# xieydd/crane-scheduler

Hardware: AMD Instinct MI355X
Metric: placements/sec (higher is better)
Workload: dtype f64

## Files before the change

crane-scheduler_amd/csrc/k1stream.hip:

```cpp
#include <hip/hip_runtime.h>

#include "k1stream_body.hpp"

namespace crane {

template <int PD, int PR, bool FULL>
__global__ __launch_bounds__(256) __attribute__((amdgpu_waves_per_eu(PD * PR <= 24 ? K1S_WAVES : 1)))
void k1_stream_steps(K1Args a, K1Step step) {
    __shared__ K1Lds<PD, PR> lds;
    k1_stream_body<PD, PR, FULL, (int)sizeof(K1Args) + (int)sizeof(K1Step)>(a, step, blockIdx.x, gridDim.x, lds);
}

template <int PD, int PR, bool FULL = false>
static hipError_t launch_t(const K1Args& a, const K1Step& sa, hipStream_t st) {
    const unsigned grid = (unsigned)((a.N + 255) / 256);
    return klaunch("k1_stream_steps", k1_stream_steps<PD, PR, FULL>, dim3(grid), dim3(256), 0, st, a, sa);
}

hipError_t launch_stream_steps(int pd, int pr, const K1Args& a, const K1Step& sa, hipStream_t st) {
    if (a.N <= 0) return hipSuccess;
    if (K1S_FULL && a.pol.npd == 4 && a.pol.npr == 6 && a.pol.n_win == kFullWin) return launch_t<4, 6, true>(a, sa, st);
    if (pd <= 4 && pr <= 6) return launch_t<4, 6>(a, sa, st);
    if (pd <= 8 && pr <= 8) return launch_t<8, 8>(a, sa, st);
    return launch_t<16, 16>(a, sa, st);
}

}
```

crane-scheduler_amd/csrc/k1stream_body.hpp:

```cpp
#pragma once
#include <hip/hip_runtime.h>

#include <cstddef>

#include "dyn_types.hpp"
#include "kernels.hpp"
#include "node_rec.hpp"
#include "step_node.hpp"

namespace crane {

#ifndef K1S_SKIP
#define K1S_SKIP 0
#endif
#ifndef K1S_TAIL1
#define K1S_TAIL1 1
#endif
#ifndef K1S_WAVES
#define K1S_WAVES 7
#endif
#ifndef K1S_KWARM
#define K1S_KWARM 1
#endif
#ifndef K1S_FULL
#define K1S_FULL 1
#endif
#ifndef K1S_SREC
#define K1S_SREC 64
#endif
#ifndef K1S_SCAP
#define K1S_SCAP 128
#endif
#ifndef K1S_RTAIL
#define K1S_RTAIL 1
#endif
#ifndef K1S_SMALL
#define K1S_SMALL 32
#endif
constexpr int kSRec = K1S_SREC;
constexpr int kSCap = K1S_SCAP;
constexpr int kSmallTail = K1S_SMALL;
static_assert(kSmallTail <= 32 && kSmallTail <= kSCap, "one record per lane of a half wave, staged in LDS");

template <int PD, int PR>
__device__ __forceinline__ void emit_task(const NodeRec<PD, PR>& r, int64_t n, int q, const int32_t* dw, int64_t tmin,
                                          int64_t tmax, double wsum, int32_t noprio, const StepTables& st,
                                          int64_t blk, const S1Out& s1o, double winv) {
    constexpr int NB = PR + 2, F = PR + 1;
    int64_t c[NB];
#pragma unroll
    for (int k = 0; k < PR; ++k) c[k] = r.e_prio[k];
    c[PR] = r.e_hv;
    c[F] = r.e_fail;
    uint32_t inm = 0;
#pragma unroll
    for (int k = 0; k < NB; ++k) inm |= (c[k] > tmin && c[k] <= tmax) ? 1u << k : 0u;
    if (!((inm >> q) & 1u)) return;
    const int cnt0 = __builtin_popcount(inm), cnt1 = __builtin_popcount(inm & ~(1u << F));
    int64_t cq = c[0];
#pragma unroll
    for (int j = 1; j < NB; ++j) cq = q == j ? c[j] : cq;
    int rk0 = 0;
    bool fb = false;
    int64_t cn1 = INT64_MAX, cn0;
#pragma unroll
    for (int j = 0; j < NB; ++j) {
        const bool in = (inm >> j) & 1u;
        const bool before = in && (c[j] < cq || (c[j] == cq && j < q));
        const bool after = in && (c[j] > cq || (c[j] == cq && j > q));
        rk0 += before;
        if (j == F) {
            fb = before;
            cn0 = after ? min(cn1, c[j]) : cn1;
        } else {
            cn1 = after ? min(cn1, c[j]) : cn1;
        }
    }
    const int rk1 = rk0 - (fb ? 1 : 0);
    double tk[PR];
#pragma unroll
    for (int k = 0; k < PR; ++k) tk[k] = r.t[k];
    double ssum = 0.0;
#pragma unroll
    for (int k = 0; k < PR; ++k) ssum = cq < c[k] ? ssum + tk[k] : ssum;
    const int64_t pk = pack_key(score_of_sum(ssum, cq < c[PR] ? r.pen : 0, wsum, noprio, winv), n);
    const int64_t pk0 = pack_key(dw[5], n);
#pragma unroll
    for (int T = 0; T < 2; ++T) {
        const int32_t slot = dw[T ? 2 : 0];
        if (slot < 0 || (T == 1 && q == F)) continue;
        const int rk = T ? rk1 : rk0, cnt = T ? cnt1 : cnt0;
        const int64_t cn = T ? cn1 : cn0;
        const int32_t kq = (int32_t)((T == 1 || !(cq < r.e_fail)) ? pk : -1);
        const int32_t kt = (int32_t)((T == 1 || !(tmin < r.e_fail)) ? pk0 : -1);
        const bool multi = ((dw[4] >> T) & 1) != 0;
        if (!multi) {
            if (rk == 0) {
                Step1 v;
                v.bp = cq;
                v.k0 = kt;
                v.k1 = kq;
                s1o.put(T, slot, v);
            }
            continue;
        }
        if (rk + 1 < cnt) {
            Mid pc;
            pc.s = cq;
            pc.e = cn;
            pc.key = kq;
            pc.pad = 0;
            (st.mid + (int64_t)T * st.mpad + blk * st.mstride + dw[T ? 3 : 1])[rk] = pc;
        }
        if (rk == 0) {
            Step1 x;
            x.bp = cq;
            x.k0 = kt;
            x.k1 = -1;
            s1o.put(T, slot, x);
        }
        if (rk == cnt - 1) {
            Step1 y;
            y.bp = cq;
            y.k0 = -1;
            y.k1 = kq;
            s1o.put(T, slot + 1, y);
        }
    }
}

template <int BS, class Rec>
__device__ __forceinline__ void tail(bool g1, Rec* lrec, Step1* s1l, Step1* srt, StepShared& ssh, const K1Step& step,
                                     int64_t blk, unsigned long long* trace, int64_t wg) {
    constexpr int kPc = ((int)(kSRec * sizeof(Rec)) / PieceScr::bytes_per_piece) & ~3;
    const PieceScr ps{reinterpret_cast<unsigned char*>(lrec), (K1S_SKIP & 8) ? 0 : (kPc < 128 ? kPc : 128)};
#if K1S_SKIP & 16
    StepTables st = step.st;
    st.rows = nullptr;
#else
    const StepTables& st = step.st;
#endif
    step_epilogue<BS, kSCap>(g1, s1l, srt, ssh, st, blk, nullptr, ps, trace, wg);
    CRANE_TSTAMP(trace, wg, 4);
}

template <bool ONE>
__device__ __forceinline__ void small_tail_bounds(const StepTables& st, int64_t (&pre)[2]) {
    const int lane = threadIdx.x & 63;
    const int T0 = ONE ? 0 : __builtin_amdgcn_readfirstlane((int)(threadIdx.x >> 6));
    pre[0] = small_tile_bound(st, T0, 0, lane);
    pre[1] = ONE ? small_tile_bound(st, 1, 0, lane) : 0;
}
template <bool ONE>
__device__ __forceinline__ void small_tail(const Step1* s1l, int32_t n0, int32_t n1, const StepShared& ssh,
                                           const K1Step& step, int64_t blk, const int64_t (&pre)[2], bool rows,
                                           unsigned long long* trace, int64_t wg) {
    constexpr int NK = ONE ? 2 : 1;
    const StepTables& st = step.st;
    const int lane = threadIdx.x & 63;
    const int T0 = ONE ? 0 : __builtin_amdgcn_readfirstlane((int)(threadIdx.x >> 6));
    const int tl = lane < 32 ? lane : 64;
    int32_t n[NK], fl[NK];
    Step1 r[NK];
    SmallScan sc[NK];
#pragma unroll
    for (int k = 0; k < NK; ++k) {
        const int T = T0 + k;
        n[k] = __builtin_amdgcn_readfirstlane(T ? n1 : n0);
        fl[k] = block_flat_max<256>(ssh, T);
        r[k].bp = 0;
        r[k].k0 = r[k].k1 = -1;
        if (lane < n[k]) r[k] = s1l[T * kSCap + lane];
    }
#pragma unroll
    for (int k = 0; k < NK; ++k) sc[k] = small_scan(r[k], n[k], lane < 32 ? r[k].bp : pre[k], tl);
#pragma unroll
    for (int k = 0; k < NK; ++k) small_records_store(T0 + k, n[k], r[k], sc[k], st, blk);
    CRANE_TSTAMP(trace, wg, 6);
    if (rows) {
#pragma unroll
        for (int k = 0; k < NK; ++k) small_row_store(T0 + k, 0, sc[k], fl[k], st, blk);
        for (int t0 = 16; t0 < st.ntiles; t0 += 16) {
#pragma unroll
            for (int k = 0; k < NK; ++k) {
                const SmallScan s = small_scan(r[k], n[k], small_tile_bound(st, T0 + k, t0, lane), 64);
                small_row_store(T0 + k, t0, s, fl[k], st, blk);
            }
        }
    }
    CRANE_TSTAMP(trace, wg, 4);
}

constexpr int kFullWin = 2;
template <int PD, int PR>
struct K1Lds {
    alignas(16) NodeRec<PD, PR> lrec[kSRec];
    alignas(16) Step1 s1l[2 * kSCap];
    alignas(16) Step1 srt[2 * kSCap];
    alignas(16) uint32_t xch[5][4];
    StepShared ssh;
    uint8_t rank_lane[256];
};
template <int PD, int PR, bool FULL, int WARM>
__device__ __forceinline__ void k1_stream_body(const K1Args& a, const K1Step& step, const int64_t wg, const int64_t nwg,
                                               K1Lds<PD, PR>& lds) {
    using Rec = NodeRec<PD, PR>;
    constexpr int BS = 256;
    const int npd = FULL ? PD : a.pol.npd, npr = FULL ? PR : a.pol.npr, nwin = FULL ? kFullWin : a.pol.n_win;
    Rec* const lrec = lds.lrec;
    uint8_t* const rank_lane = lds.rank_lane;
    Step1* const s1l = lds.s1l;
    Step1* const srt = lds.srt;
    uint32_t(*const xch)[4] = lds.xch;
    StepShared& ssh = lds.ssh;
    const DevPolicy& pol = a.pol;
    const int64_t N = a.N;
    const int64_t blk = xcd_block(wg, nwg), first = blk * BS, n = first + threadIdx.x;
    CRANE_TSTAMP(a.trace, wg, 0);
    const int lo = (int)min((int64_t)threadIdx.x, N - 1 - first);
    const int64_t bt0 = step.batch[0], bt1 = step.batch[1];
    int64_t pt[PD], qt[PR];
    double pv[PD], qv[PR];
#pragma unroll
    for (int k = 0; k < PD; ++k) {
        pt[k] = kTsInvalid;
        pv[k] = 0.0;
    }
#pragma unroll
    for (int k = 0; k < PR; ++k) {
        qt[k] = kTsInvalid;
        qv[k] = 0.0;
    }
    if (FULL || pol.n_slots > 0) {
#pragma unroll
        for (int k = 0; k < PD; ++k) {
            const int64_t row = k < npd ? pol.pred_slot[k] : 0;
            pt[k] = (a.ts + (row * N + first))[lo];
            pv[k] = (a.val + (row * N + first))[lo];
        }
#pragma unroll
        for (int k = 0; k < PR; ++k) {
            const int64_t row = k < npr ? pol.prio_slot[k] : 0;
            qt[k] = (a.ts + (row * N + first))[lo];
            qv[k] = (a.val + (row * N + first))[lo];
        }
    }
    uint32_t bc[kMaxWin];
    double hvl = 0.0;
    int64_t hvt = kTsInvalid;
    if (a.buckets) {
        const uint32_t* __restrict__ base = a.bucket_base ? a.bucket_base : a.buckets;
        uint32_t bz[kMaxWin];
#pragma unroll
        for (int b = 0; b < kMaxWin; ++b) {
            bc[b] = b < nwin ? (a.buckets + first)[(int64_t)b * N + lo] : 0u;
            bz[b] = b < nwin ? (base + first)[(int64_t)b * N + lo] : 0u;
        }
        if (a.bucket_base) bucket_anchor_counts(bz, bc);
    } else if (a.hv) {
        hvl = a.hv[first + lo];
        hvt = a.hv_ts ? a.hv_ts[first + lo] : a.hv_ts_counts;
    }
#if K1S_KWARM
    kernarg_warm<WARM>();
#endif
    const int64_t tmin = readfirstlane64(bt0), tmax = readfirstlane64(bt1);
    if (threadIdx.x < 4) ssh.lc[threadIdx.x >> 1][threadIdx.x & 1] = 0;
    CRANE_TSTAMP(a.trace, wg, 1);
    const bool valid = n < N;
    int64_t e_fail = kTsInvalid;
#pragma unroll
    for (int k = 0; k < PD; ++k) {
        const double u = pv[k], lim = pol.pred_limit[k];
        const int64_t e = sat_add(pt[k], pol.pred_dur[k]);
        const bool over = k < npd && pt[k] != kTsInvalid && !(u < 0.0) && lim != 0.0 && u > lim;
        e_fail = over ? max(e_fail, e) : e_fail;
    }
    Rec hr;
    if (a.buckets) {
        if (valid && !a.buckets_keep) {
#pragma unroll
            for (int b = 0; b < kMaxWin; ++b)
                if (b < nwin) (a.buckets + first)[(int64_t)b * N + threadIdx.x] = 0;
        }
        rec_hot_counts<PD, PR, FULL ? kFullWin : 0>(pol, bc, N, n, valid ? a.cnt_out : nullptr, valid ? a.hvc_out : nullptr,
                               a.hv_ts_counts, hr);
    } else if (a.hv) {
        rec_hot_annotation<PD, PR>(hvl, hvt, hr);
    } else {
        hr.pen = 0;
        hr.e_hv = kTsInvalid;
    }
    double s = 0.0;
    StepRange both;
    int64_t ep[PR];
    double tp[PR];
#pragma unroll
    for (int k = 0; k < PR; ++k) {
        const bool use = k < npr && qt[k] != kTsInvalid && !(qv[k] < 0.0);
        double term = (1.0 - qv[k]) * pol.prio_w[k];
        term = term * 100.0;
        const int64_t e = sat_add(qt[k], pol.prio_dur[k]);
        ep[k] = use ? e : kTsInvalid;
        tp[k] = use ? term : 0.0;
        s = tmin < ep[k] ? s + tp[k] : s;
        both.add(ep[k], tmin, tmax);
    }
    both.add(hr.e_hv, tmin, tmax);
    const int32_t s0 = score_of_sum(s, tmin < hr.e_hv ? hr.pen : 0, step.wsum, step.noprio, step.winv);
    StepRange g[2];
    StepSlots so;
    step_classify(both, e_fail, valid, s0, n, tmin, tmax, g, so);
    CRANE_TSTAMP(a.trace, wg, 2);
    const int lane = threadIdx.x & 63, wv = threadIdx.x >> 6;
    const uint32_t w0 = g[0].word(), w1 = g[1].word(), w2 = (g[0].cnt | g[1].cnt) ? 1u : 0u;
    uint32_t e0 = wave_scan_add(w0), e1 = wave_scan_add(w1), e2 = wave_scan_add(w2);
    const int32_t fm0 = wave_max(so.flat0), fm1 = wave_max(so.flat1);
    if (lane == 0) {
        ssh.fm[0][wv] = fm0;
        ssh.fm[1][wv] = fm1;
    }
    if (lane == 63) {
        xch[0][wv] = e0;
        xch[1][wv] = e1;
        xch[2][wv] = e2;
    }
    e0 -= w0;
    e1 -= w1;
    e2 -= w2;
    __syncthreads();
    uint32_t base[3], tot[3];
#pragma unroll
    for (int k = 0; k < 3; ++k) {
        const uint4 x = *reinterpret_cast<const uint4*>(xch[k]);
        base[k] = (wv > 0 ? x.x : 0u) + (wv > 1 ? x.y : 0u) + (wv > 2 ? x.z : 0u);
        tot[k] = x.x + x.y + x.z + x.w;
    }
    step_slots(g, base[0] + e0, base[1] + e1, so);
    const int32_t rs = (int32_t)(base[2] + e2);
    const int32_t nst = (int32_t)tot[2];
    if (threadIdx.x == 0) {
        ssh.lc[0][0] = (int32_t)(tot[0] & 0xFFFF);
        ssh.lc[0][1] = (int32_t)(tot[0] >> 16);
        ssh.lc[1][0] = (int32_t)(tot[1] & 0xFFFF);
        ssh.lc[1][1] = (int32_t)(tot[1] >> 16);
    }
    step_publish_store<BS>(ssh, step.st, blk, [&](int L) {
        return (int32_t)((L & 1) ? tot[L >> 1] >> 16 : tot[L >> 1] & 0xFFFF);
    });
    const bool g1 = (int32_t)max(tot[0] & 0xFFFF, tot[1] & 0xFFFF) > min(kSCap, step.st.lds_cap);
    CRANE_TSTAMP(a.trace, wg, 3);
    const S1Out s1o{s1l, step.st.stage + blk * 2 * step.st.bs, g1, (int64_t)kSCap, step.st.s1pad};
    const bool stepped = (g[0].cnt | g[1].cnt) != 0;
    auto put = [&](Rec* r) {
        r->e_fail = e_fail;
        r->pen = hr.pen;
        r->e_hv = hr.e_hv;
#pragma unroll
        for (int k = 0; k < PR; ++k) {
            r->e_prio[k] = ep[k];
            r->t[k] = tp[k];
        }
        int32_t* dw = reinterpret_cast<int32_t*>(r->e_pred);
        dw[0] = so.slot0;
        dw[1] = so.mslot0;
        dw[2] = so.slot1;
        dw[3] = so.mslot1;
        dw[4] = (so.multi0 ? 1 : 0) | (so.multi1 ? 2 : 0);
        dw[5] = s0;
    };
    if (stepped && !(K1S_SKIP & 4)) {
        rank_lane[rs] = (uint8_t)threadIdx.x;
        if (rs < kSRec) put(&lrec[rs]);
        else put(static_cast<Rec*>(step.srec) + n);
    }
    __syncthreads();
    const bool t1 = K1S_TAIL1 && (step.tail1 == 1 || (step.tail1 == 0 && nwg >= 4096));
    const bool emit1 = t1 && nst * (PR + 2) <= 64;
    if (emit1 && threadIdx.x >= 64) return;
    const int nthr = emit1 ? 64 : BS;
#if K1S_RTAIL
    const int32_t n0 = (int32_t)(tot[0] & 0xFFFF), n1 = (int32_t)(tot[1] & 0xFFFF);
    const bool small = !g1 && max(n0, n1) <= kSmallTail && !step.st.prow && !(K1S_SKIP & 2);
    const bool srows = step.st.rows && !(K1S_SKIP & 16);
    int64_t tpre[2] = {0, 0};
    if (small && srows && threadIdx.x < (t1 ? 64 : 128)) {
        if (t1) small_tail_bounds<true>(step.st, tpre);
        else small_tail_bounds<false>(step.st, tpre);
    }
#endif
    for (int32_t c0 = 0; c0 < ((K1S_SKIP & 1) ? 0 : nst); c0 += kSRec) {
        const int32_t m = min(kSRec, nst - c0);
        if (c0 > 0) {
            constexpr int W = 3 + 2 * PR + 3;
            for (int i = threadIdx.x; i < m * W; i += BS) {
                const int j = i / W, f = i - j * W;
                const int64_t* src = reinterpret_cast<const int64_t*>(static_cast<const Rec*>(step.srec) + first +
                                                                      rank_lane[c0 + j]);
                reinterpret_cast<int64_t*>(&lrec[j])[f] = src[f];
            }
            __syncthreads();
        }
        {
            constexpr int NB = PR + 2;
            for (int tk = threadIdx.x; tk < m * NB; tk += nthr) {
                const int j = tk / NB;
                int q = tk - j * NB;
                asm volatile("" : "+v"(q));
                emit_task<PD, PR>(lrec[j], first + rank_lane[c0 + j], q,
                                  reinterpret_cast<const int32_t*>(lrec[j].e_pred), tmin, tmax, step.wsum, step.noprio,
                                  step.st, blk, s1o, step.winv);
            }
        }
        __syncthreads();
    }
    CRANE_TSTAMP(a.trace, wg, 5);
    if (K1S_SKIP & 2) return;
#if K1S_RTAIL
    if (small) {
        if (threadIdx.x >= (t1 ? 64 : 128)) return;
        if (t1) small_tail<true>(s1l, n0, n1, ssh, step, blk, tpre, srows, a.trace, wg);
        else small_tail<false>(s1l, n0, n1, ssh, step, blk, tpre, srows, a.trace, wg);
        return;
    }
#endif
    if (t1) {
        if (threadIdx.x >= 64) return;
        if (threadIdx.x < 2) {
            const int T = threadIdx.x;
            ssh.fm[T][0] = block_flat_max<BS>(ssh, T);
        }
        tail<64>(g1, lrec, s1l, srt, ssh, step, blk, a.trace, wg);
        return;
    }
    tail<BS>(g1, lrec, s1l, srt, ssh, step, blk, a.trace, wg);
}

}
```

crane-scheduler_amd/csrc/lds_hash.hpp:

```cpp
#pragma once
#include <hip/hip_runtime.h>

#include <cstdint>

#include "kernels.hpp"

namespace crane {

constexpr int kDSlots = 4096;

template <int SLOTS = kDSlots>
__device__ __forceinline__ int32_t hash_add(int32_t* hkey, uint32_t* hcnt, uint32_t* hist, int bb, int32_t key,
                                            uint32_t add) {
    constexpr int kBits = __builtin_ctz(SLOTS);
    uint32_t h = ((uint32_t)key * 2654435761u) >> (32 - kBits);
    for (;;) {
        const int32_t old = atomicCAS(&hkey[h], -1, key);
        if (old == -1 || old == key) {
            atomicAdd(&hcnt[h], add);
            if (old == -1) {
                atomicAdd(&hist[(key >> 3) >> bb], 1u);
                return (int32_t)h;
            }
            return -1;
        }
        h = (h + 1) & (SLOTS - 1);
    }
}

template <int SLOTS, int KPER>
__device__ __forceinline__ uint32_t wave_aggregate(const int32_t* key, int32_t* hkey, uint32_t* hcnt, uint32_t* hist,
                                                   int bb, uint16_t* useg) {
    const int lane = threadIdx.x & 63;
    uint32_t nw = 0;
#pragma unroll
    for (int u = 0; u < KPER; ++u) {
        const bool ok = key[u] >= 0;
        const uint64_t am = __ballot(ok);
        if (am == 0) continue;
        const int lead = __ffsll((long long)am) - 1;
        const int32_t kl = __builtin_amdgcn_readlane(key[u], lead);
        const uint64_t m = __ballot(ok && key[u] == kl);
        const bool mine = lane == lead || (ok && key[u] != kl);
        const int32_t slot = mine ? hash_add<SLOTS>(hkey, hcnt, hist, bb, lane == lead ? kl : key[u],
                                                    lane == lead ? (uint32_t)__popcll(m) : 1u)
                                  : -1;
        const uint64_t nm = __ballot(slot >= 0);
        if (slot >= 0) useg[nw + __popcll(nm & ((1ull << lane) - 1ull))] = (uint16_t)slot;
        nw += __popcll(nm);
    }
    return nw;
}

constexpr int kDeltaChunk = 1024;
constexpr int delta_slots(int chunk) { return 2 * kDeltaMaxWin * chunk; }
constexpr size_t delta_lds_bytes(int chunk, int threads) {
    return sizeof(uint32_t) * 2 * (size_t)delta_slots(chunk) +
           sizeof(uint16_t) * (size_t)(threads / 64) * (size_t)(chunk / threads * kDeltaMaxWin * 64);
}

template <int BT, int CHUNK = kDeltaChunk>
__device__ __forceinline__ void k2_delta_body(const int32_t blk, const int32_t* __restrict__ bnode, int64_t N,
                                              const HotDelta& d, uint32_t* __restrict__ adj) {
    static_assert(CHUNK % BT == 0 && BT % 64 == 0, "whole bindings per lane, whole waves");
    constexpr int kSlots = delta_slots(CHUNK);
    static_assert((kSlots & (kSlots - 1)) == 0 && kSlots <= 65536, "hash_add masks the slot; uniq holds it in 16 bits");
    constexpr int kPer = CHUNK / BT;
    constexpr int kKeys = kPer * kDeltaMaxWin;
    static_assert(sizeof(uint32_t) * 2 * (size_t)kSlots + sizeof(uint16_t) * (BT / 64) * (kKeys * 64) ==
                      delta_lds_bytes(CHUNK, BT),
                  "the launchers' footprint is this layout's");
    extern __shared__ __attribute__((aligned(16))) uint32_t sh[];
    __shared__ uint32_t hist[32];
    int32_t* hkey = reinterpret_cast<int32_t*>(sh);
    uint32_t* hcnt = sh + kSlots;
    uint16_t* uniq = reinterpret_cast<uint16_t*>(hcnt + kSlots);
    const int64_t L = d.start[d.n_rng];
    int64_t pos[kPer];
    int32_t nd[kPer];
#pragma unroll
    for (int u = 0; u < kPer; ++u) {
        const int64_t t = (int64_t)blk * CHUNK + u * BT + threadIdx.x;
        int k = 0;
        for (int r = 1; r < d.n_rng; ++r) k += t >= d.start[r] ? 1 : 0;
        pos[u] = d.lo[k] + (t - d.start[k]);
        nd[u] = bnode[t < L ? pos[u] : d.lo[0]];
        if (t >= L) nd[u] = -1;
    }
    for (int i = threadIdx.x; i < kSlots; i += BT) {
        hkey[i] = -1;
        hcnt[i] = 0;
    }
    if (threadIdx.x < 32) hist[threadIdx.x] = 0;
    __syncthreads();
    int32_t key[kKeys];
#pragma unroll
    for (int u = 0; u < kPer; ++u) {
        const bool ok = nd[u] >= 0 && (int64_t)nd[u] < N;
#pragma unroll
        for (int r = 0; r < kDeltaMaxWin; ++r) {
            const bool ia = pos[u] >= d.a[r], ip = pos[u] >= d.p[r];
            key[u * kDeltaMaxWin + r] = ok && r < d.n_win && ia != ip ? ((nd[u] * 8 + r) << 1) | (ia ? 1 : 0) : -1;
        }
    }
    uint16_t* useg = uniq + (threadIdx.x >> 6) * (kKeys * 64);
    const uint32_t nw = wave_aggregate<kSlots, kKeys>(key, hkey, hcnt, hist, 24, useg);
    __syncthreads();
    for (uint32_t i = threadIdx.x & 63; i < nw; i += 64) {
        const int s = useg[i];
        const int32_t k = hkey[s];
        const uint32_t c = hcnt[s];
        atomicAdd(&adj[(int64_t)((k >> 1) & 7) * N + (k >> 4)], (k & 1) ? 0u - c : c);
    }
}


}
```

crane-scheduler_amd/csrc/pods.hpp:

```cpp
#pragma once
#include <hip/hip_runtime.h>

#include <cstdint>

#include "kernels.hpp"

namespace crane {

constexpr size_t kK3pLds = 1024 * (sizeof(uint64_t) + sizeof(uint32_t));

__device__ __forceinline__ bool pod_gt(uint64_t ka, uint32_t va, uint64_t kb, uint32_t vb) {
    return (va >> 30) != (vb >> 30) ? va > vb : (ka != kb ? ka > kb : va > vb);
}

template <int kT>
__device__ __forceinline__ void k3p_tile(const int64_t t, const PodPrep& pp, unsigned char* lds) {
    static_assert(1024 % kT == 0 && kT >= 64, "a tile is 1024 pods");
    constexpr int kU = 1024 / kT, kG = kU * (kT / 64);
    constexpr uint64_t kSign = 1ull << 63;
    __shared__ int32_t gcn[kG], gcd[kG];
    uint64_t* ku = reinterpret_cast<uint64_t*>(lds);
    uint32_t* kv = reinterpret_cast<uint32_t*>(lds + 8 * 1024);
    const int w = threadIdx.x >> 6, lane = threadIdx.x & 63;
    const int64_t pend = min(pp.P, (t + 1) * 1024);
    bool live[kU], ds[kU], inorder = true;
    int64_t tn[kU];
#pragma unroll
    for (int u = 0; u < kU; ++u) {
        const int64_t p = t * 1024 + u * kT + threadIdx.x;
        live[u] = p < pend;
        ds[u] = live[u] && pp.flags && (pp.flags[p] & 1u);
        tn[u] = live[u] ? pp.now[p] : 0;
        if (p + 1 < pend) inorder &= tn[u] <= pp.now[p + 1];
        if (live[u] && pp.keys) pp.keys[p] = -1;
    }
    int32_t e0, e1;
    if (__syncthreads_and(inorder)) {
        uint64_t mnm[kU], mdm[kU];
#pragma unroll
        for (int u = 0; u < kU; ++u) {
            mnm[u] = __ballot(live[u] && !ds[u]);
            mdm[u] = __ballot(ds[u]);
            if (lane == 0) {
                gcn[u * (kT / 64) + w] = __popcll(mnm[u]);
                gcd[u * (kT / 64) + w] = __popcll(mdm[u]);
            }
        }
        __syncthreads();
        int32_t tot_n = 0, tot_d = 0;
#pragma unroll
        for (int i = 0; i < kG; ++i) {
            tot_n += gcn[i];
            tot_d += gcd[i];
        }
        e0 = tot_n;
        e1 = tot_n + tot_d;
        const uint64_t lt = (1ull << lane) - 1ull;
#pragma unroll
        for (int u = 0; u < kU; ++u) {
            const int gi = u * (kT / 64) + w, i = u * kT + threadIdx.x;
            int32_t pre_n = 0, pre_d = 0;
            for (int k = 0; k < gi; ++k) {
                pre_n += gcn[k];
                pre_d += gcd[k];
            }
            const int pos = !live[u] ? i
                            : ds[u]  ? tot_n + pre_d + __popcll(mdm[u] & lt)
                                     : pre_n + __popcll(mnm[u] & lt);
            ku[pos] = live[u] ? (uint64_t)tn[u] ^ kSign : ~0ull;
            kv[pos] = ((live[u] ? (ds[u] ? 1u : 0u) : 2u) << 30) | (uint32_t)i;
        }
        __syncthreads();
    } else {
        e0 = e1 = 0;
#pragma unroll
        for (int u = 0; u < kU; ++u) {
            const int i = u * kT + threadIdx.x;
            ku[i] = live[u] ? (uint64_t)tn[u] ^ kSign : ~0ull;
            kv[i] = ((live[u] ? (ds[u] ? 1u : 0u) : 2u) << 30) | (uint32_t)i;
            e0 += __syncthreads_count(live[u] && !ds[u]);
            e1 += __syncthreads_count(ds[u]);
        }
        e1 += e0;
        for (int k = 2; k <= 1024; k <<= 1) {
            for (int j = k >> 1; j > 0; j >>= 1) {
                for (int q = threadIdx.x; q < 512; q += kT) {
                    const int i = ((q & ~(j - 1)) << 1) | (q & (j - 1)), l = i | j;
                    const uint64_t ka = ku[i], kb = ku[l];
                    const uint32_t va = kv[i], vb = kv[l];
                    if (pod_gt(ka, va, kb, vb) == ((i & k) == 0)) {
                        ku[i] = kb;
                        ku[l] = ka;
                        kv[i] = vb;
                        kv[l] = va;
                    }
                }
                __syncthreads();
            }
        }
    }
#pragma unroll
    for (int u = 0; u < kU; ++u) {
        const int i = u * kT + threadIdx.x;
        const uint32_t v = kv[i];
        if ((v >> 30) < 2u) {
            pp.perm[t * 1024 + i] = (int32_t)(t * 1024 + (v & 1023u)) | ((v >> 30) ? (int32_t)0x80000000 : 0);
            pp.pnow[t * 1024 + i] = (int64_t)(ku[i] ^ kSign);
        }
    }
    if (threadIdx.x == 0) {
        int64_t* ts = pp.tile_mm + kTileStat * t;
        const int64_t n0 = e0 > 0 ? (int64_t)(ku[0] ^ kSign) : INT64_MAX;
        const int64_t x0 = e0 > 0 ? (int64_t)(ku[e0 - 1] ^ kSign) : INT64_MIN;
        const int64_t n1 = e1 > e0 ? (int64_t)(ku[e0] ^ kSign) : INT64_MAX;
        const int64_t x1 = e1 > e0 ? (int64_t)(ku[e1 - 1] ^ kSign) : INT64_MIN;
        ts[0] = n0;
        ts[1] = x0;
        ts[2] = n1;
        ts[3] = x1;
        ts[4] = e0;
        ts[5] = e1 - e0;
        if (pp.batch) {
            if (t == 0) {
                pp.batch_next[0] = INT64_MAX;
                pp.batch_next[1] = INT64_MIN;
            }
            const int64_t mn = min(n0, n1), mx = max(x0, x1);
            if (mn != INT64_MAX) __hip_atomic_fetch_min(&pp.batch[0], mn, __ATOMIC_RELAXED, __HIP_MEMORY_SCOPE_AGENT);
            if (mx != INT64_MIN) __hip_atomic_fetch_max(&pp.batch[1], mx, __ATOMIC_RELAXED, __HIP_MEMORY_SCOPE_AGENT);
        }
    }
}

}
```

crane-scheduler_amd/csrc/step.hip:

```cpp
#include <hip/hip_runtime.h>

#include <algorithm>

#include "dyn_types.hpp"
#include "kernels.hpp"
#include "pods.hpp"
#include "lds_hash.hpp"
#include "step_node.hpp"
#include "k1stream_body.hpp"

#ifndef K3S_BUCKETS
#define K3S_BUCKETS 1
#endif
#ifndef K3_KWARM
#define K3_KWARM 1
#endif

namespace crane {

constexpr int kPodTile = 1024;

__global__ __launch_bounds__(kPodTile) void k3p_pods(PodPrep pp) {
    extern __shared__ __attribute__((aligned(16))) unsigned char lds[];
    k3p_tile<kPodTile>(blockIdx.x, pp, lds);
// ... 184 lines not shown
    CRANE_TSTAMP(st.trace, b, 5);
    const int32_t n1[2] = {any[0] ? c.x : 0, any[1] ? c.z : 0};
    const int32_t pl[2] = {st.prow ? prow.x & 0xFFFF : 0, st.prow ? prow.y & 0xFFFF : 0};
    const int32_t nm[2] = {any[0] ? (st.prow ? (prow.x >> 16) - pl[0] : c.y) : 0,
                           any[1] ? (st.prow ? (prow.y >> 16) - pl[1] : c.w) : 0};
    const Step1* base[2] = {st.single + s1_at(st, 0, ob), st.single + s1_at(st, 1, ob)};
    int32_t jj[4] = {0, 0, 0, 0};
    int32_t um[2] = {-1, -1};
    if (st.rows) {
        if (own) {
            jj[0] = row.z & 0xFFFF;
            jj[1] = row.z >> 16;
            jj[2] = row.w & 0xFFFF;
            jj[3] = row.w >> 16;
            if (sub == 0) {
                um[0] = row.x;
                um[1] = row.y;
            }
        }
    } else {
        if (own) team_count_le(base[0], base[1], n1, tlo, thi, sub, lpb, lead, jj);
        if (own && sub == 0) {
#pragma unroll
            for (int T = 0; T < 2; ++T) {
                if (!any[T]) continue;
                const int64_t o = s1_at(st, T, ob);
                int32_t u = st.flat[ob * 2 + T];
                if (jj[2 * T] > 0) u = max(u, st.pm1[o + jj[2 * T] - 1]);
                if (jj[2 * T + 1] < n1[T]) u = max(u, st.sm0[o + jj[2 * T + 1]]);
                um[T] = u;
            }
        }
    }
    const bool lists = m <= kK3sListBlk;
    if (lists && own && sub == 0) {
        wpre[2 * j + 0] = max(0, jj[1] - jj[0]);
        wpre[2 * j + 1] = max(0, jj[3] - jj[2]);
        wpre[2 * m + 2 * j + 0] = nm[0];
        wpre[2 * m + 2 * j + 1] = nm[1];
        wjl[2 * j] = jj[0];
        wjl[2 * j + 1] = jj[2];
        wpl[2 * j] = pl[0];
        wpl[2 * j + 1] = pl[1];
    }
    __syncthreads();
    CRANE_TSTAMP(st.trace, b, 1);
    const int32_t E = 4 * m;
    auto bucket_table = [&]() {
#if K3S_BUCKETS
        static_assert(2 * kSearchBuckets % TH == 0, "whole rounds over (kind, bucket)");
#pragma unroll
        for (int q = threadIdx.x; q < 2 * kSearchBuckets; q += TH) {
            const int T = q / kSearchBuckets, k = q % kSearchBuckets;
            if (klo[T] < khi[T]) {
                sfirst[T][k] = slot_lower(tt, klo[T], khi[T], tlo[T] + ((int64_t)k << sbs[T]));
                if (k == 0) sfirst[T][kSearchBuckets] = khi[T];
            }
        }
#endif
    };
    int32_t nrec = 0, total = 0;
    if (lists) {
        if (threadIdx.x < 64) {
            const int32_t v = lane < E ? wpre[lane] : 0;
            int32_t carry = (int32_t)wave_scan_add((uint32_t)v);
            if (lane < E) wpre[lane] = carry - v;
            carry = __builtin_amdgcn_readlane(carry, 63);
            for (int32_t e0 = 64; e0 < E; e0 += 64) {
                const int32_t e = e0 + lane;
                const int32_t x = e < E ? wpre[e] : 0;
                const int32_t inc = (int32_t)wave_scan_add((uint32_t)x) + carry;
                if (e < E) wpre[e] = inc - x;
                carry = __builtin_amdgcn_readlane(inc, 63);
            }
            if (lane == 0) wpre[E] = carry;
        }
        bucket_table();
        __syncthreads();
        nrec = wpre[2 * m];
        total = wpre[E];
    } else if (K3S_BUCKETS) {
        bucket_table();
        __syncthreads();
    }
    const bool piece_list = lists && total - nrec <= kK3sPieceList;
    const bool rec_list = lists && nrec <= kK3sRecList;
    bool upd = false;
    const int32_t i0 = rec_list ? 0 : nrec, i1 = piece_list ? total : nrec;
    if (i1 > i0) {
        for (int32_t e = threadIdx.x; e < E; e += TH) {
            const int32_t a = max(wpre[e], i0), z = min(wpre[e + 1], i1);
            for (int32_t i = a; i < z; ++i) imap[i - i0] = (uint8_t)e;
        }
        __syncthreads();
        constexpr int kU = 2, kPass = (kK3sRecList + kK3sPieceList) / (kU * TH);
#pragma unroll
        for (int h = 0; h < kPass; ++h) {
            if (i0 + h * kU * TH >= i1) break;
            Step1 r1[kU];
            Mid pm[kU];
            int32_t ee[kU];
#pragma unroll
            for (int u = 0; u < kU; ++u) {
                const int32_t it = i0 + (h * kU + u) * TH + (int32_t)threadIdx.x;
                ee[u] = -1;
                if (it >= i1) continue;
                const int32_t e = imap[it - i0];
                ee[u] = e;
                const bool rec = e < 2 * m;
                const int32_t ej = rec ? e : e - 2 * m, jb = ej >> 1, T = ej & 1, idx = it - wpre[e];
                const int64_t obj = xc + (int64_t)stride * (k0 + jb);
                if (rec) r1[u] = (st.single + s1_at(st, T, obj))[wjl[2 * jb + T] + idx];
                else pm[u] = st.mid[(int64_t)T * st.mpad + obj * st.mstride + wpl[ej] + idx];
            }
#pragma unroll
            for (int u = 0; u < kU; ++u) {
                const int32_t e = ee[u];
                if (e < 0) continue;
                const bool rec = e < 2 * m;
                const int T = (rec ? e : e - 2 * m) & 1;
                if (rec) {
                    const int32_t sp = find(T, r1[u].bp);
                    if (r1[u].k0 >= 0) tree_max(tree, klo[T], sp, r1[u].k0);
                    if (r1[u].k1 >= 0) tree_max(tree, sp, khi[T], r1[u].k1);
                    upd = true;
                } else {
                    const Mid& q = pm[u];
                    if (q.s <= tlo[T] && q.e > thi[T]) um[T] = max(um[T], q.key);
                    else if (q.s <= thi[T] && q.e > tlo[T]) {
                        tree_max(tree, find(T, q.s), find(T, q.e), q.key);
                        upd = true;
                    }
                }
            }
        }
    }
    if (own && !rec_list) {
#pragma unroll
        for (int T = 0; T < 2; ++T) {
            for (int32_t i = jj[2 * T] + sub; i < jj[2 * T + 1]; i += lpb) {
                const Step1 q = base[T][i];
                const int32_t sp = find(T, q.bp);
                if (q.k0 >= 0) tree_max(tree, klo[T], sp, q.k0);
                if (q.k1 >= 0) tree_max(tree, sp, khi[T], q.k1);
                upd = true;
            }
        }
    }
    CRANE_TSTAMP(st.trace, b, 6);
    if (own && !piece_list) {
#pragma unroll
        for (int T = 0; T < 2; ++T) {
            const Mid* mp = st.mid + (int64_t)T * st.mpad + ob * st.mstride + pl[T];
            for (int32_t i0 = sub; i0 < nm[T]; i0 += 4 * lpb) {
                Mid q[4];
#pragma unroll
                for (int v = 0; v < 4; ++v) {
                    const int32_t i = i0 + v * lpb;
                    if (i < nm[T]) q[v] = mp[i];
                    else q[v].s = INT64_MAX;
                }
#pragma unroll
                for (int v = 0; v < 4; ++v) {
                    const Mid& pm = q[v];
                    if (pm.s <= tlo[T] && pm.e > thi[T]) um[T] = max(um[T], pm.key);
                    else if (pm.s <= thi[T] && pm.e > tlo[T]) {
                        tree_max(tree, find(T, pm.s), find(T, pm.e), pm.key);
                        upd = true;
                    }
                }
            }
        }
    }
    CRANE_TSTAMP(st.trace, b, 2);
#pragma unroll
    for (int T = 0; T < 2; ++T) {
        um[T] = wave_max(um[T]);
        if (lane == 0 && um[T] >= 0) atomicMax(&umax[T], um[T]);
    }
    const bool tree_used = __syncthreads_or(upd);
    CRANE_TSTAMP(st.trace, b, 3);
    constexpr int kLevels = 11;
    static_assert(kK3sPods == 1 << (kLevels - 1), "a segment tree over the tile's 1024 slots");
    constexpr int kV = 2;
    static_assert(kPPL % kV == 0, "whole passes");
#pragma unroll
    for (int h = 0; h < kPPL / kV; ++h) {
        int32_t anc[kV][kLevels];
        if (tree_used) {
#pragma unroll
            for (int v = 0; v < kV; ++v)
#pragma unroll
                for (int l = 0; l < kLevels; ++l)
                    anc[v][l] = tree[((h * kV + v) * TH + threadIdx.x + kK3sPods) >> l];
        }
#pragma unroll
        for (int v = 0; v < kV; ++v) {
            const int u = h * kV + v;
            int32_t best = umax[praw[u] < 0 ? 1 : 0];
            if (tree_used) {
#pragma unroll
                for (int l = 0; l < kLevels; ++l) best = max(best, anc[v][l]);
            }
            const bool live = grp * kK3sPods + u * TH + threadIdx.x < P;
            if (live && best >= 0) {
                const int64_t sc = best >> 24;
                const int64_t n = 0xFFFFFF - (best & 0xFFFFFF);
                atomicMax(&keys[praw[u] & 0x7FFFFFFF],
                          (long long)((sc << 32) | (int64_t)(0xFFFFFFFFull - (uint64_t)(node_offset + n))));
            }
        }
        if (h + 1 < kPPL / kV) asm volatile("" ::: "memory");
    }
    CRANE_TSTAMP(st.trace, b, 4);
}

int step_breakpoints(int shape) {
    switch (shape) {
        case kShape4x6: return 6 + 2;
        case kShape8x8: return 8 + 2;
        default: return 16 + 2;
    }
}

__global__ __launch_bounds__(kK3sThreads) void k3s_eval(StepTables st, const int32_t* __restrict__ perm,
                                                        const int64_t* __restrict__ pnow,
                                                        const int64_t* __restrict__ tile_mm, int64_t P,
                                                        int64_t node_offset, int32_t R,
                                                        long long* __restrict__ keys) {
#if K3_KWARM
    kernarg_warm<(int)sizeof(StepTables) + 64>();
#endif
    __shared__ K3sLds lds;
    k3s_body<kK3sThreads>((int64_t)blockIdx.x, st, perm, pnow, tile_mm, P, node_offset, R, keys, lds);
}

struct K3sArgs {
    StepTables st;
    const int32_t* perm;
    const int64_t* pnow;
    const int64_t* tile_mm;
    int64_t P, node_offset;
    int32_t R;
    long long* keys;
};
static_assert(kK3sThreads == 512, "the fused launch's workgroups are the delta form's and K3p's 512 lanes");

__global__ __launch_bounds__(kK3sThreads) void k3s_delta_pods(K3sArgs k, int32_t nk3s, const int32_t* __restrict__ bnode,
                                                              int64_t N, HotDelta d, uint32_t* __restrict__ adj,
                                                              PodPrep pp) {
#if K3_KWARM
    kernarg_warm<(int)(sizeof(K3sArgs) + 32 + sizeof(HotDelta) + 8 + sizeof(PodPrep))>();
#endif
    const int64_t b = blockIdx.x;
    if (b < nk3s) {
        __shared__ K3sLds lds;
        k3s_body<kK3sThreads>(b, k.st, k.perm, k.pnow, k.tile_mm, k.P, k.node_offset, k.R, k.keys, lds);
        return;
    }
    extern __shared__ __attribute__((aligned(16))) unsigned char dyn_lds[];
    if (b - nk3s < pp.ntiles) k3p_tile<kK3sThreads>(b - nk3s, pp, dyn_lds);
    else k2_delta_body<kK3sThreads>((int32_t)(b - nk3s - pp.ntiles), bnode, N, d, adj);
}

struct KeyReset {
    long long* keys;
    int64_t P;
};
constexpr int kStepOneThreads = 256;
constexpr int kResetPerWg = 4 * kStepOneThreads;
static_assert(kResetPerWg == kPodTile, "step_one_workgroups counts a reset workgroup per pod tile");
constexpr size_t kStepOneDeltaLds = delta_lds_bytes(kStepOneDeltaChunk, kStepOneThreads);
constexpr size_t cmax(size_t a, size_t b) { return a > b ? a : b; }
constexpr size_t kStepOneLds = cmax(cmax(sizeof(K1Lds<4, 6>), sizeof(K3sLds)), cmax(kK3pLds, kStepOneDeltaLds));
static_assert(kStepOneLds >= sizeof(K1Lds<4, 6>) && kStepOneLds >= sizeof(K3sLds) && kStepOneLds >= kK3pLds &&
                  kStepOneLds >= kStepOneDeltaLds,
              "the union holds the largest body");
static_assert(kStepOneLds == sizeof(K3sLds), "no body asks for more than K3s");
static_assert(7 * (kStepOneLds + 512) <= 160 * 1024, "seven workgroups per compute unit (160 KiB)");
const int kStepOneWgPerCu =
    (int)std::min<size_t>(160 * 1024 / (kStepOneLds + 512), 4 * (K1S_WAVES - 1) / (kStepOneThreads / 64));
constexpr int kOneK3sEnd = (int)sizeof(K3sArgs) + 16;
constexpr int kOneK1End = kOneK3sEnd + (int)sizeof(KeyReset) + (int)sizeof(K1Args) + (int)sizeof(K1Step) + 8;
constexpr int kOneEnd = kOneK1End + 16 + (int)sizeof(HotDelta) + 8 + (int)sizeof(PodPrep);

template <bool FULL>
__global__ __launch_bounds__(kStepOneThreads) __attribute__((amdgpu_waves_per_eu(FULL ? K1S_WAVES : K1S_WAVES - 1)))
void step_one_launch(K3sArgs k, int32_t nk3s, int32_t nk1, int32_t nk1pad, int32_t nreset, KeyReset kr, K1Args a,
                     K1Step step, const int32_t* __restrict__ bnode, int64_t N, HotDelta d, uint32_t* __restrict__ adj,
                     PodPrep pp) {
    extern __shared__ __attribute__((aligned(16))) unsigned char dyn_lds[];
    int64_t b = blockIdx.x;
    if (b < nk3s) {
#if K3_KWARM
        kernarg_warm<kOneK3sEnd>();
#endif
        k3s_body<kStepOneThreads>(b, k.st, k.perm, k.pnow, k.tile_mm, k.P, k.node_offset, k.R, k.keys,
                                  *reinterpret_cast<K3sLds*>(dyn_lds));
        return;
    }
    b -= nk3s;
    if (b < nk1pad) {
        if (b >= nk1) return;
        k1_stream_body<4, 6, FULL, kOneK1End>(a, step, b, nk1, *reinterpret_cast<K1Lds<4, 6>*>(dyn_lds));
        return;
    }
    b -= nk1pad;
    if (b < nreset) {
#pragma unroll
        for (int u = 0; u < kResetPerWg / kStepOneThreads; ++u) {
            const int64_t p = b * kResetPerWg + u * kStepOneThreads + threadIdx.x;
            if (p < kr.P) kr.keys[p] = -1;
        }
        return;
    }
    b -= nreset;
#if K3_KWARM
    kernarg_warm<kOneEnd, kOneK1End>();
#endif
    if (b < pp.ntiles) k3p_tile<kStepOneThreads>(b, pp, dyn_lds);
    else k2_delta_body<kStepOneThreads, kStepOneDeltaChunk>((int32_t)(b - pp.ntiles), bnode, N, d, adj);
}

__global__ __launch_bounds__(256) void keys_reset(long long* __restrict__ keys, int64_t P) {
    const int64_t p = (int64_t)blockIdx.x * 256 + threadIdx.x;
    if (p < P) keys[p] = -1;
}

StepGeometry step_geometry(int64_t P, int64_t N, int32_t nblk, int32_t blk_per_wg) {
    StepGeometry g{};
    g.nseg = (N + kStepSeg - 1) / kStepSeg;
    g.npad = g.nseg * kStepSeg;
    g.ntiles = (P + kPodTile - 1) / kPodTile;
    g.ngroups = (P + kK3sPods - 1) / kK3sPods;
    constexpr int64_t kMaxWg = 2048;
    const int32_t bpw = blk_per_wg > 0 ? blk_per_wg : kK3sBlkPerWg;
    int64_t R = (std::max<int32_t>(nblk, 1) + bpw - 1) / bpw;
    if (blk_per_wg <= 0) R = std::min<int64_t>(R, std::max<int64_t>(1, kMaxWg / std::max<int64_t>(g.ngroups, 1)));
    R = std::max<int64_t>(R, (nblk + kK3sMaxBlk - 1) / kK3sMaxBlk);
    if (nblk >= 8) {
        R = (R + 7) / 8 * 8;
        if (blk_per_wg <= 0 && R * g.ngroups > kMaxWg) R -= 8;
        R = std::max<int64_t>(8, R);
        while (((nblk + 7) / 8 + R / 8 - 1) / (R / 8) > kK3sMaxBlk) R += 8;
    }
    g.R = (int32_t)R;
    return g;
}

template <int PD, int PR>
static hipError_t launch_steps_t(const void* rec, int64_t N, double wsum, int32_t noprio, const StepTables& st,
                                 const StepGeometry& g, const int64_t* tile_mm, hipStream_t s) {
    return klaunch("k3a_steps", k3a_steps<PD, PR>, dim3((unsigned)g.nseg), dim3(kStepSeg), 0, s,
                   static_cast<const NodeRec<PD, PR>*>(rec), N, tile_mm, (int32_t)g.ntiles, wsum, noprio, st);
}

hipError_t launch_step_pods(const int64_t* now, const uint8_t* flags, int64_t P, long long* keys, int64_t* batch,
                            int64_t* batch_next, const StepGeometry& g, int32_t* perm, int64_t* pnow,
                            int64_t* tile_mm, hipStream_t s) {
    if (P <= 0) return hipSuccess;
    const PodPrep pp{now, flags, P, g.ntiles, perm, pnow, tile_mm, keys, batch, batch_next};
    return klaunch("k3p_pods", k3p_pods, dim3((unsigned)g.ntiles), dim3(kPodTile), kK3pLds, s, pp);
}

hipError_t launch_step_nodes(int shape, const void* rec, int64_t N, double wsum, int32_t noprio,
                             const StepTables& st, const StepGeometry& g, const int64_t* tile_mm, hipStream_t s) {
    if (N <= 0 || g.ntiles <= 0) return hipSuccess;
    if (N >= kStepMaxNodes) return hipErrorInvalidValue;
    switch (shape) {
        case kShape4x6: return launch_steps_t<4, 6>(rec, N, wsum, noprio, st, g, tile_mm, s);
        case kShape8x8: return launch_steps_t<8, 8>(rec, N, wsum, noprio, st, g, tile_mm, s);
        default: return launch_steps_t<16, 16>(rec, N, wsum, noprio, st, g, tile_mm, s);
    }
}

hipError_t launch_k3s_delta_pods(const K3sBatch& b, const int32_t* bnode, int64_t N, const HotDelta& d, uint32_t* adj,
                                 const PodPrep& pods, hipStream_t s) {
    if (b.P <= 0 || b.N <= 0 || d.n_win < 1 || d.n_win > kDeltaMaxWin || d.n_rng < 0 || d.n_rng > kMaxWin ||
        N >= (1LL << 27))
        return hipErrorInvalidValue;
    const int64_t nk = b.g.ngroups * b.g.R;
    const int64_t L = d.n_rng > 0 ? d.start[d.n_rng] : 0;
    const int64_t grid = nk + (pods.P > 0 ? pods.ntiles : 0) + (L + kDeltaChunk - 1) / kDeltaChunk;
    if (grid >= (1LL << 31) || nk >= (1LL << 31)) return hipErrorInvalidValue;
    PodPrep pp{};
    if (pods.P > 0) pp = pods;
    constexpr size_t lds = cmax(kK3pLds, delta_lds_bytes(kDeltaChunk, kK3sThreads));
    static_assert(lds + sizeof(K3sLds) <= 64 * 1024, "beside K3s's static LDS in a workgroup's 64 KiB");
    static const hipError_t attr = hipFuncSetAttribute((const void*)k3s_delta_pods,
                                                       hipFuncAttributeMaxDynamicSharedMemorySize, (int)lds);
    if (attr != hipSuccess) return attr;
    const K3sArgs k{b.st, b.perm, b.pnow, b.tile_mm, b.P, b.node_offset, b.g.R, b.keys};
    return klaunch("k3s_eval+k2_delta+k3p_pods", k3s_delta_pods, dim3((unsigned)grid), dim3(kK3sThreads), lds, s, k,
                   (int32_t)nk, bnode, N, d, adj, pp);
}

bool step_one_has(int shape) { return shape == kShape4x6; }

int64_t step_one_workgroups(int64_t nk3s, int64_t N_k1, int64_t ntiles, int64_t delta_len) {
    const int64_t nk1 = (N_k1 + 255) / 256;
    return nk3s + (nk1 + 7) / 8 * 8 + 2 * ntiles + (delta_len + kStepOneDeltaChunk - 1) / kStepOneDeltaChunk;
}

hipError_t launch_step_one(const StepOne& s, hipStream_t st) {
    const bool k3s = s.k3s && s.k3s->P > 0 && s.k3s->N > 0, k1 = s.k1 && s.ks && s.k1->N > 0;
    const bool delta = s.d != nullptr, pods = s.pods && s.pods->P > 0;
    if (delta && (s.d->n_win < 1 || s.d->n_win > kDeltaMaxWin || s.d->n_rng < 0 || s.d->n_rng > kMaxWin ||
                  s.N >= (1LL << 27)))
        return hipErrorInvalidValue;
    if (k1 && (s.k1->threads != 256 || s.k1->out || s.k1->hx_region || !s.ks->st.stage)) return hipErrorInvalidValue;
    const int64_t nk = k3s ? s.k3s->g.ngroups * s.k3s->g.R : 0;
    const int64_t nk1 = k1 ? (s.k1->N + 255) / 256 : 0, nk1pad = (nk1 + 7) / 8 * 8;
    const int64_t L = delta && s.d->n_rng > 0 ? s.d->start[s.d->n_rng] : 0;
    const KeyReset kr{s.reset_keys, k1 && s.reset_keys && s.reset_P > 0 ? s.reset_P : 0};
    const int64_t nreset = (kr.P + kResetPerWg - 1) / kResetPerWg;
    const int64_t grid = nk + nk1pad + nreset + (pods ? s.pods->ntiles : 0) +
                         (L + kStepOneDeltaChunk - 1) / kStepOneDeltaChunk;
    if (grid >= (1LL << 31)) return hipErrorInvalidValue;
    if (grid == 0) return hipSuccess;
    const K3sBatch kb = k3s ? *s.k3s : K3sBatch{};
    const K3sArgs k{kb.st, kb.perm, kb.pnow, kb.tile_mm, kb.P, kb.node_offset, kb.g.R, kb.keys};
    const K1Args a = k1 ? *s.k1 : K1Args{};
    const K1Step ks = k1 ? *s.ks : K1Step{};
    const HotDelta d = delta ? *s.d : HotDelta{};
    const PodPrep pp = pods ? *s.pods : PodPrep{};
    const bool full = K1S_FULL && k1 && a.pol.npd == 4 && a.pol.npr == 6 && a.pol.n_win == kFullWin;
    static const hipError_t attr[2] = {
        hipFuncSetAttribute((const void*)step_one_launch<false>, hipFuncAttributeMaxDynamicSharedMemorySize,
                            (int)kStepOneLds),
        hipFuncSetAttribute((const void*)step_one_launch<true>, hipFuncAttributeMaxDynamicSharedMemorySize,
                            (int)kStepOneLds)};
    if (attr[full] != hipSuccess) return attr[full];
    const char* nm = "k3s_eval+k1_stream_steps+k2_delta+k3p_pods";
    return full ? klaunch(nm, step_one_launch<true>, dim3((unsigned)grid), dim3(kStepOneThreads), kStepOneLds, st, k,
                          (int32_t)nk, (int32_t)nk1, (int32_t)nk1pad, (int32_t)nreset, kr, a, ks, s.bnode, s.N, d, s.adj, pp)
                : klaunch(nm, step_one_launch<false>, dim3((unsigned)grid), dim3(kStepOneThreads), kStepOneLds, st, k,
                          (int32_t)nk, (int32_t)nk1, (int32_t)nk1pad, (int32_t)nreset, kr, a, ks, s.bnode, s.N, d, s.adj, pp);
}

hipError_t launch_keys_reset(long long* keys, int64_t P, hipStream_t st) {
    if (P <= 0 || !keys) return hipSuccess;
    return klaunch("keys_reset", keys_reset, dim3((unsigned)((P + 255) / 256)), dim3(256), 0, st, keys, P);
}

hipError_t launch_step_pairs(const K3sBatch& b, hipStream_t s) {
    if (b.P <= 0 || b.N <= 0) return hipSuccess;
    const dim3 grid((unsigned)(b.g.ngroups * b.g.R)), blk(kK3sThreads);
    return klaunch("k3s_eval", k3s_eval, grid, blk, 0, s, b.st, b.perm, b.pnow, b.tile_mm, b.P, b.node_offset, b.g.R,
                   b.keys);
}

}
```

Measured before the change: 2.393 billion.

## Hoist kernargs into scalar registers and batch loads ahead of dependent logic

Reads kernel arguments and slot indices into a head struct that is pinned to scalar registers through empty asm constraints, and casts pointers to the global address space so the compiler can emit global loads instead of flat loads. Annotation and bucket loads in the FULL path are issued before the kernarg warm and the anchor fix-up. The pod tile loads flags and now values up front in a separate loop, and the delta body replaces its per-thread range search loop with predicated unrolled selects. All of this aims to expose more memory-level parallelism and cut load latency stalls, at the cost of added SGPR pressure and some redundant loads.

Result: no change. 2.399 billion, median of 4 (+0.2%).

```diff
diff --git a/crane-scheduler_amd/csrc/k1stream.hip b/crane-scheduler_amd/csrc/k1stream.hip
--- a/crane-scheduler_amd/csrc/k1stream.hip
+++ b/crane-scheduler_amd/csrc/k1stream.hip
@@ -8,7 +8,8 @@
 __global__ __launch_bounds__(256) __attribute__((amdgpu_waves_per_eu(PD * PR <= 24 ? K1S_WAVES : 1)))
 void k1_stream_steps(K1Args a, K1Step step) {
     __shared__ K1Lds<PD, PR> lds;
-    k1_stream_body<PD, PR, FULL, (int)sizeof(K1Args) + (int)sizeof(K1Step)>(a, step, blockIdx.x, gridDim.x, lds);
+    const K1Head<PD, PR> h = k1_head<PD, PR, FULL>(a, step);
+    k1_stream_body<PD, PR, FULL, (int)sizeof(K1Args) + (int)sizeof(K1Step)>(a, step, h, blockIdx.x, gridDim.x, lds);
 }
 
 template <int PD, int PR, bool FULL = false>
diff --git a/crane-scheduler_amd/csrc/k1stream_body.hpp b/crane-scheduler_amd/csrc/k1stream_body.hpp
--- a/crane-scheduler_amd/csrc/k1stream_body.hpp
+++ b/crane-scheduler_amd/csrc/k1stream_body.hpp
@@ -201,12 +201,61 @@
     StepShared ssh;
     uint8_t rank_lane[256];
 };
+template <class T>
+using gptr = T __attribute__((address_space(1)))*;
+template <int PD, int PR>
+struct K1Head {
+    int64_t N;
+    gptr<const int64_t> ts;
+    gptr<const double> val;
+    gptr<uint32_t> buckets;
+    gptr<const uint32_t> bucket_base;
+    gptr<const double> hv;
+    gptr<const int64_t> hv_ts;
+    gptr<const int64_t> batch;
+    gptr<unsigned long long> trace;
+    int32_t n_slots, npd, npr, nwin;
+    int32_t pred_slot[PD], prio_slot[PR];
+};
+template <int PD, int PR, bool FULL>
+__device__ __forceinline__ K1Head<PD, PR> k1_head(const K1Args& a, const K1Step& step) {
+    K1Head<PD, PR> h;
+    h.N = a.N;
+    h.ts = (gptr<const int64_t>)a.ts;
+    h.val = (gptr<const double>)a.val;
+    h.buckets = (gptr<uint32_t>)a.buckets;
+    h.bucket_base = (gptr<const uint32_t>)a.bucket_base;
+    h.hv = (gptr<const double>)a.hv;
+    h.hv_ts = (gptr<const int64_t>)a.hv_ts;
+    h.batch = (gptr<const int64_t>)step.batch;
+    h.trace = (gptr<unsigned long long>)a.trace;
+    h.n_slots = FULL ? 1 : a.pol.n_slots;
+    h.npd = FULL ? PD : a.pol.npd;
+    h.npr = FULL ? PR : a.pol.npr;
+    h.nwin = FULL ? kFullWin : a.pol.n_win;
+#pragma unroll
+    for (int k = 0; k < PD; ++k) h.pred_slot[k] = a.pol.pred_slot[k];
+#pragma unroll
+    for (int k = 0; k < PR; ++k) h.prio_slot[k] = a.pol.prio_slot[k];
+    asm volatile(""
+                 : "+s"(h.N), "+s"(h.ts), "+s"(h.val), "+s"(h.buckets), "+s"(h.bucket_base), "+s"(h.hv), "+s"(h.hv_ts),
+                   "+s"(h.batch), "+s"(h.trace));
+    if constexpr (PD == 4 && PR == 6) {
+        int32_t* const p = h.pred_slot;
+        int32_t* const q = h.prio_slot;
+        asm volatile(""
+                     : "+s"(p[0]), "+s"(p[1]), "+s"(p[2]), "+s"(p[3]), "+s"(q[0]), "+s"(q[1]), "+s"(q[2]), "+s"(q[3]),
+                       "+s"(q[4]), "+s"(q[5]));
+    }
+    return h;
+}
+
 template <int PD, int PR, bool FULL, int WARM>
-__device__ __forceinline__ void k1_stream_body(const K1Args& a, const K1Step& step, const int64_t wg, const int64_t nwg,
-                                               K1Lds<PD, PR>& lds) {
+__device__ __forceinline__ void k1_stream_body(const K1Args& a, const K1Step& step, const K1Head<PD, PR>& h,
+                                               const int64_t wg, const int64_t nwg, K1Lds<PD, PR>& lds) {
     using Rec = NodeRec<PD, PR>;
     constexpr int BS = 256;
-    const int npd = FULL ? PD : a.pol.npd, npr = FULL ? PR : a.pol.npr, nwin = FULL ? kFullWin : a.pol.n_win;
+    const int npd = FULL ? PD : h.npd, npr = FULL ? PR : h.npr, nwin = FULL ? kFullWin : h.nwin;
     Rec* const lrec = lds.lrec;
     uint8_t* const rank_lane = lds.rank_lane;
     Step1* const s1l = lds.s1l;
@@ -214,11 +263,11 @@
     uint32_t(*const xch)[4] = lds.xch;
     StepShared& ssh = lds.ssh;
     const DevPolicy& pol = a.pol;
-    const int64_t N = a.N;
+    const int64_t N = h.N;
     const int64_t blk = xcd_block(wg, nwg), first = blk * BS, n = first + threadIdx.x;
-    CRANE_TSTAMP(a.trace, wg, 0);
+    CRANE_TSTAMP(h.trace, wg, 0);
     const int lo = (int)min((int64_t)threadIdx.x, N - 1 - first);
-    const int64_t bt0 = step.batch[0], bt1 = step.batch[1];
+    const int64_t bt0 = h.batch[0], bt1 = h.batch[1];
     int64_t pt[PD], qt[PR];
     double pv[PD], qv[PR];
 #pragma unroll
@@ -231,39 +280,51 @@
         qt[k] = kTsInvalid;
         qv[k] = 0.0;
     }
-    if (FULL || pol.n_slots > 0) {
+    if (FULL || h.n_slots > 0) {
 #pragma unroll
         for (int k = 0; k < PD; ++k) {
-            const int64_t row = k < npd ? pol.pred_slot[k] : 0;
-            pt[k] = (a.ts + (row * N + first))[lo];
-            pv[k] = (a.val + (row * N + first))[lo];
+            const int64_t row = k < npd ? h.pred_slot[k] : 0;
+            pt[k] = (h.ts + (row * N + first))[lo];
+            pv[k] = (h.val + (row * N + first))[lo];
         }
 #pragma unroll
         for (int k = 0; k < PR; ++k) {
-            const int64_t row = k < npr ? pol.prio_slot[k] : 0;
-            qt[k] = (a.ts + (row * N + first))[lo];
-            qv[k] = (a.val + (row * N + first))[lo];
-        }
-    }
-    uint32_t bc[kMaxWin];
+            const int64_t row = k < npr ? h.prio_slot[k] : 0;
+            qt[k] = (h.ts + (row * N + first))[lo];
+            qv[k] = (h.val + (row * N + first))[lo];
+        }
+    }
+    uint32_t bc[kMaxWin], bz[kMaxWin];
     double hvl = 0.0;
     int64_t hvt = kTsInvalid;
-    if (a.buckets) {
-        const uint32_t* __restrict__ base = a.bucket_base ? a.bucket_base : a.buckets;
-        uint32_t bz[kMaxWin];
+    bool hvt_counts = false;
+    auto load_annotation = [&]() {
+        hvl = h.hv[first + lo];
+        if (h.hv_ts) hvt = h.hv_ts[first + lo];
+        else hvt_counts = true;
+    };
+    auto load_buckets = [&]() {
+        const gptr<const uint32_t> base = h.bucket_base ? h.bucket_base : (gptr<const uint32_t>)h.buckets;
 #pragma unroll
         for (int b = 0; b < kMaxWin; ++b) {
-            bc[b] = b < nwin ? (a.buckets + first)[(int64_t)b * N + lo] : 0u;
+            bc[b] = b < nwin ? (h.buckets + first)[(int64_t)b * N + lo] : 0u;
             bz[b] = b < nwin ? (base + first)[(int64_t)b * N + lo] : 0u;
         }
-        if (a.bucket_base) bucket_anchor_counts(bz, bc);
-    } else if (a.hv) {
-        hvl = a.hv[first + lo];
-        hvt = a.hv_ts ? a.hv_ts[first + lo] : a.hv_ts_counts;
+    };
+    if (FULL) {
+        if (!h.buckets && h.hv) load_annotation();
+        if (h.buckets) load_buckets();
+    } else if (h.buckets) {
+        load_buckets();
+        if (h.bucket_base) bucket_anchor_counts(bz, bc);
+    } else if (h.hv) {
+        load_annotation();
     }
 #if K1S_KWARM
     kernarg_warm<WARM>();
 #endif
+    if (hvt_counts) hvt = a.hv_ts_counts;
+    if (FULL && h.buckets && h.bucket_base) bucket_anchor_counts(bz, bc);
     const int64_t tmin = readfirstlane64(bt0), tmax = readfirstlane64(bt1);
     if (threadIdx.x < 4) ssh.lc[threadIdx.x >> 1][threadIdx.x & 1] = 0;
     CRANE_TSTAMP(a.trace, wg, 1);
@@ -277,15 +338,15 @@
         e_fail = over ? max(e_fail, e) : e_fail;
     }
     Rec hr;
-    if (a.buckets) {
+    if (h.buckets) {
         if (valid && !a.buckets_keep) {
 #pragma unroll
             for (int b = 0; b < kMaxWin; ++b)
-                if (b < nwin) (a.buckets + first)[(int64_t)b * N + threadIdx.x] = 0;
+                if (b < nwin) (h.buckets + first)[(int64_t)b * N + threadIdx.x] = 0;
         }
         rec_hot_counts<PD, PR, FULL ? kFullWin : 0>(pol, bc, N, n, valid ? a.cnt_out : nullptr, valid ? a.hvc_out : nullptr,
                                a.hv_ts_counts, hr);
-    } else if (a.hv) {
+    } else if (h.hv) {
         rec_hot_annotation<PD, PR>(hvl, hvt, hr);
     } else {
         hr.pen = 0;
diff --git a/crane-scheduler_amd/csrc/lds_hash.hpp b/crane-scheduler_amd/csrc/lds_hash.hpp
--- a/crane-scheduler_amd/csrc/lds_hash.hpp
+++ b/crane-scheduler_amd/csrc/lds_hash.hpp
@@ -75,18 +75,28 @@
     int32_t* hkey = reinterpret_cast<int32_t*>(sh);
     uint32_t* hcnt = sh + kSlots;
     uint16_t* uniq = reinterpret_cast<uint16_t*>(hcnt + kSlots);
-    const int64_t L = d.start[d.n_rng];
+    const int32_t nrng = d.n_rng;
+    int64_t L = d.start[0];
+#pragma unroll
+    for (int r = 1; r <= kMaxWin; ++r) L = r == nrng ? d.start[r] : L;
     int64_t pos[kPer];
     int32_t nd[kPer];
 #pragma unroll
     for (int u = 0; u < kPer; ++u) {
         const int64_t t = (int64_t)blk * CHUNK + u * BT + threadIdx.x;
-        int k = 0;
-        for (int r = 1; r < d.n_rng; ++r) k += t >= d.start[r] ? 1 : 0;
-        pos[u] = d.lo[k] + (t - d.start[k]);
+        int64_t lo = d.lo[0], st = d.start[0];
+#pragma unroll
+        for (int r = 1; r < kMaxWin; ++r) {
+            const bool in = r < nrng && t >= d.start[r];
+            lo = in ? d.lo[r] : lo;
+            st = in ? d.start[r] : st;
+        }
+        pos[u] = lo + (t - st);
         nd[u] = bnode[t < L ? pos[u] : d.lo[0]];
-        if (t >= L) nd[u] = -1;
     }
+#pragma unroll
+    for (int u = 0; u < kPer; ++u)
+        if ((int64_t)blk * CHUNK + u * BT + threadIdx.x >= L) nd[u] = -1;
     for (int i = threadIdx.x; i < kSlots; i += BT) {
         hkey[i] = -1;
         hcnt[i] = 0;
diff --git a/crane-scheduler_amd/csrc/pods.hpp b/crane-scheduler_amd/csrc/pods.hpp
--- a/crane-scheduler_amd/csrc/pods.hpp
+++ b/crane-scheduler_amd/csrc/pods.hpp
@@ -25,14 +25,31 @@
     const int64_t pend = min(pp.P, (t + 1) * 1024);
     bool live[kU], ds[kU], inorder = true;
     int64_t tn[kU];
+    uint8_t fb[kU];
+    int64_t tx[kU];
+    const bool has_flags = pp.flags != nullptr;
+    const uint8_t* const fp = has_flags ? pp.flags : reinterpret_cast<const uint8_t*>(pp.now);
+#pragma unroll
+    for (int u = 0; u < kU; ++u) {
+        const int64_t p = t * 1024 + u * kT + threadIdx.x;
+        int64_t pn = min(p + 1, pend - 1);
+        asm volatile("" : "+v"(pn));
+        fb[u] = fp[min(p, pend - 1)];
+        tn[u] = pp.now[min(p, pend - 1)];
+        tx[u] = pp.now[pn];
+    }
 #pragma unroll
     for (int u = 0; u < kU; ++u) {
         const int64_t p = t * 1024 + u * kT + threadIdx.x;
         live[u] = p < pend;
-        ds[u] = live[u] && pp.flags && (pp.flags[p] & 1u);
-        tn[u] = live[u] ? pp.now[p] : 0;
-        if (p + 1 < pend) inorder &= tn[u] <= pp.now[p + 1];
-        if (live[u] && pp.keys) pp.keys[p] = -1;
+        ds[u] = live[u] && has_flags && (fb[u] & 1u);
+        if (!live[u]) tn[u] = 0;
+        if (p + 1 < pend) inorder &= tn[u] <= tx[u];
+    }
+    if (pp.keys) {
+#pragma unroll
+        for (int u = 0; u < kU; ++u)
+            if (live[u]) pp.keys[t * 1024 + u * kT + threadIdx.x] = -1;
     }
     int32_t e0, e1;
     if (__syncthreads_and(inorder)) {
diff --git a/crane-scheduler_amd/csrc/step.hip b/crane-scheduler_amd/csrc/step.hip
--- a/crane-scheduler_amd/csrc/step.hip
+++ b/crane-scheduler_amd/csrc/step.hip
@@ -510,7 +510,8 @@
     b -= nk3s;
     if (b < nk1pad) {
         if (b >= nk1) return;
-        k1_stream_body<4, 6, FULL, kOneK1End>(a, step, b, nk1, *reinterpret_cast<K1Lds<4, 6>*>(dyn_lds));
+        const K1Head<4, 6> kh = k1_head<4, 6, FULL>(a, step);
+        k1_stream_body<4, 6, FULL, kOneK1End>(a, step, kh, b, nk1, *reinterpret_cast<K1Lds<4, 6>*>(dyn_lds));
         return;
     }
     b -= nk1pad;
```
